# Nesquiko/Latticeum

Measured on AMD Instinct MI355X. Metric: fold-steps/sec (Ajtai commit+fold) at d=1024, higher is better.
Workload: dtype u64 (Goldilocks mod-p integer); 1 GPU; configs[2] at d=1024: commit+fold step, X^1024+1, W=16384, kappa=32, K=15; rho is an input; transcript, linearization, sumchecks, Mz outside the step; d=1024, W=16384, N=81920, kappa=32

## Files before the change

### latticeum_amd/csrc/ajtai_mfma.hip

```cpp
#include <cstdlib>
#include <cstring>

#include "frag.hpp"
#include "kernels.hpp"
#include "launch.hpp"

namespace lfk {

int mfma_dim(int d) { return d == 24 ? 40 : d; }

FragGeom frag_geom(size_t ncols, int Lp) {
  FragGeom g;
  g.Lp = Lp;
  g.Wp = ncols / Lp;
  const size_t nG = frag_groups(g.Wp);
  g.ptop = (int)frag_ptop(nG, Lp);
  g.nch = (int)(frag_npos(nG, Lp) / 2);
  return g;
}

template <bool VMAJOR, bool PHI72, bool ONEROW>
__global__ void __launch_bounds__(256) k_to_frag(VecPtrs rows, int rlo, int rhi, int d, int dv, int nch, int Lp,
                                                 size_t Wp, uint4 *frag, int qd) {
  __shared__ uint64_t tile[TF_R * TF_S * TF_J];
  const int sb = blockIdx.x, tid = threadIdx.x;
  const int c0 = ONEROW ? blockIdx.y * TF_R : blockIdx.y;
  const int r0 = ONEROW ? rlo : (rlo & ~(TF_R - 1)) + blockIdx.z * TF_R;
  if (PHI72) {
    const int r = tid >> 5, j = tid & 31;
    const int c = ONEROW ? c0 + r : c0, row = ONEROW ? r0 : r0 + r;
    bool ok;
    const size_t col = frag_column(c, j, Lp, Wp, ok);
    uint64_t ev[TF_S];
#pragma unroll
    for (int i = 0; i < TF_S; i++) ev[i] = 0;
    if (row >= rlo && row < rhi && c < nch && ok) {
      const uint64_t *e = rows.p[row] + col * d;
      if (sb == 0)
        phi72_evals<0>(e, ev);
      else if (sb == 1)
        phi72_evals<1>(e, ev);
      else
        phi72_evals<2>(e, ev);
    }
#pragma unroll
    for (int i = 0; i < TF_S; i++) tile[(r * TF_S + i) * TF_J + j] = VMAJOR ? fenc(ev[i]) : d8(ev[i]);
  } else {
#pragma unroll
    for (int it = 0; it < TF_R * 32 * 8 / 256; it++) {
      const int p = it * 256 + tid;
      const int r = p >> 8, j = (p >> 3) & 31, q = p & 7;
      const int c = ONEROW ? c0 + r : c0, row = ONEROW ? r0 : r0 + r;
      bool ok;
      const size_t col = frag_column(c, j, Lp, Wp, ok);
      ulonglong2 v = make_ulonglong2(0, 0);
      if (row >= rlo && row < rhi && c < nch && ok)
        v = *reinterpret_cast<const ulonglong2 *>(rows.p[row] + col * d + sb * TF_S + 2 * q);
      uint64_t *t = tile + (r * TF_S + 2 * q) * TF_J + j;
      t[0] = VMAJOR ? fenc(v.x) : d8(v.x);
      t[TF_J] = VMAJOR ? fenc(v.y) : d8(v.y);
    }
  }
  __syncthreads();
  const int r = tid & 7, h = (tid >> 3) & 1, sl = tid >> 4;
  const int c = ONEROW ? c0 + r : c0, row = ONEROW ? r0 : r0 + r;
  if (row < rlo || row >= rhi || c >= nch || sb * TF_S + sl >= dv) return;
  const ulonglong2 *src = reinterpret_cast<const ulonglong2 *>(tile + (r * TF_S + sl) * TF_J + 16 * h);
  uint64_t x[16];
#pragma unroll
  for (int q = 0; q < 8; q++) {
    const ulonglong2 t = src[q];
    x[2 * q] = t.x;
    x[2 * q + 1] = t.y;
  }
  uint4 u[8];
  d8_transpose16(x, u);
  const size_t s = op_slot((size_t)sb * TF_S + sl, qd);
  if (VMAJOR) {
    uint4 *out = frag + fv_index(s, nch, c, row, h);
#pragma unroll
    for (int b = 0; b < 8; b++) out[4 * b] = u[b];
  } else {
    uint4 *out = frag + ((s * nch + c) * 8) * 64 + row + 32 * h;
#pragma unroll
    for (int b = 0; b < 8; b++) out[b * 64] = u[b];
  }
}

constexpr int AJ_CPS = 320;
typedef __attribute__((address_space(3))) void lds_void;
__device__ __forceinline__ int fl_pi(int j, int i) { return i ^ (((j & 7) << 1) | ((i >> 5) & 1)); }

__device__ __forceinline__ void mfma_epilogue(const v16i *acc, int lane, int kt, int kappa, int nvec, int d, int so,
                                              int js, int direct, const OutPtrs &dst, uint64_t *partial,
                                              const uint64_t *kr) {
  const int v = lane & 31, h = lane >> 5;
  auto fe = [](int64_t x) { return x < 0 ? (uint64_t)x + gl::P : (uint64_t)x; };
#pragma unroll
  for (int i = 0; i < 16; i++) {
    int32_t x[15];
#pragma unroll
    for (int t = 0; t < 15; t++) x[t] = acc[t][i];
    asm volatile("" : "+v"(x[0]), "+v"(x[1]), "+v"(x[2]), "+v"(x[3]), "+v"(x[4]), "+v"(x[5]), "+v"(x[6]), "+v"(x[7]),
                 "+v"(x[8]), "+v"(x[9]), "+v"(x[10]), "+v"(x[11]), "+v"(x[12]), "+v"(x[13]), "+v"(x[14]));
    int64_t S[4] = {0, 0, 0, 0};
#pragma unroll
    for (int t = 0; t < 15; t++) S[t >> 2] += (int64_t)x[t] << (8 * (t & 3));
    uint64_t r = gl::add(fe(S[0] - S[2] - S[3]), gl::mul_pow2(fe(S[1] + S[2]), 32));
    const int row = 32 * kt + (i & 3) + 8 * (i >> 2) + 4 * h;
    if (v < nvec && row < kappa) {
      if (js == 0) r = gl::add(r, kr[(size_t)row * d + so]);
      if (direct)
        dst.p[v][(size_t)row * d + so] = r;
      else
        partial[(((size_t)js * nvec + v) * kappa + row) * d + so] = r;
    }
  }
}
__device__ __forceinline__ void mfma_epilogue_top(const v16i *acc, int lane, int kt, int kappa, int d, int so,
                                                  bool add_kr, uint64_t *out, const uint64_t *kr) {
  const int h = lane >> 5;
  auto fe = [](int64_t x) { return x < 0 ? (uint64_t)x + gl::P : (uint64_t)x; };
#pragma unroll
  for (int i = 0; i < 16; i++) {
    int32_t x[15];
#pragma unroll
    for (int t = 0; t < 15; t++) x[t] = acc[t][i];
    asm volatile("" : "+v"(x[0]), "+v"(x[1]), "+v"(x[2]), "+v"(x[3]), "+v"(x[4]), "+v"(x[5]), "+v"(x[6]), "+v"(x[7]),
                 "+v"(x[8]), "+v"(x[9]), "+v"(x[10]), "+v"(x[11]), "+v"(x[12]), "+v"(x[13]), "+v"(x[14]));
    int64_t S[4] = {0, 0, 0, 0};
#pragma unroll
    for (int t = 0; t < 15; t++) S[t >> 2] += (int64_t)x[t] << (8 * (t & 3));
    uint64_t r = gl::add(fe(S[0] - S[2] - S[3]), gl::mul_pow2(fe(S[1] + S[2]), 32));
    const int row = 32 * kt + (i & 3) + 8 * (i >> 2) + 4 * h;
    if (out && row < kappa) {
      if (add_kr) r = gl::add(r, kr[(size_t)row * d + so]);
      out[(size_t)row * d + so] = r;
    }
  }
}

template <int N>
__device__ __forceinline__ void vm_wait() {
  static_assert(N >= 0 && N < 64, "vmcnt is 6 bits");
  asm volatile("s_waitcnt vmcnt(%0)" ::"n"(N) : "memory");
}
template <int DP>
__device__ __forceinline__ void vm_wait_chunk(int nf) {
  switch (nf) {
    case 8: vm_wait<8 + (DP - 2) * 16>(); break;
    case 7: vm_wait<8 + (DP - 2) * 15>(); break;
    case 6: vm_wait<8 + (DP - 2) * 14>(); break;
    case 5: vm_wait<8 + (DP - 2) * 13>(); break;
    case 4: vm_wait<8 + (DP - 2) * 12>(); break;
    case 3: vm_wait<8 + (DP - 2) * 11>(); break;
    case 2: vm_wait<8 + (DP - 2) * 10>(); break;
    case 1: vm_wait<8 + (DP - 2) * 9>(); break;
    default: vm_wait<8 + (DP - 2) * 8>(); break;
  }
}
__device__ __forceinline__ void lgkm_wait_digit(int kb) {
  switch (kb) {
    case 0: asm volatile("s_waitcnt lgkmcnt(7)" ::: "memory"); break;
    case 1: asm volatile("s_waitcnt lgkmcnt(6)" ::: "memory"); break;
    case 2: asm volatile("s_waitcnt lgkmcnt(5)" ::: "memory"); break;
    case 3: asm volatile("s_waitcnt lgkmcnt(4)" ::: "memory"); break;
    case 4: asm volatile("s_waitcnt lgkmcnt(3)" ::: "memory"); break;
    case 5: asm volatile("s_waitcnt lgkmcnt(2)" ::: "memory"); break;
    case 6: asm volatile("s_waitcnt lgkmcnt(1)" ::: "memory"); break;
    default: asm volatile("s_waitcnt lgkmcnt(0)" ::: "memory"); break;
  }
}
template <int CPOL>
__device__ __forceinline__ v4i gload16(const v4i *p) {
  v4i r;
  if (CPOL == 2)
    asm volatile("global_load_dwordx4 %0, %1, off nt" : "=v"(r) : "v"(p) : "memory");
  else
    asm volatile("global_load_dwordx4 %0, %1, off" : "=v"(r) : "v"(p) : "memory");
  return r;
}
template <class T>
__device__ __forceinline__ T *uniform_ptr(T *p) {
  const uint64_t x = (uint64_t)(uintptr_t)p;
  const uint32_t lo = __builtin_amdgcn_readfirstlane((uint32_t)x), hi = __builtin_amdgcn_readfirstlane((uint32_t)(x >> 32));
  return reinterpret_cast<T *>((uintptr_t)(((uint64_t)hi << 32) | lo));
}
template <int CPA, int CPF, int DP, bool TOP>
__global__ void __launch_bounds__(256, 1) k_ajtai_mfma_ra(const uint4 *Af, const uint64_t *kr, StepOps so_, int nsteps,
                                                         int d, int nch,
                                                         int nvec, int kappa, int direct, int cps, int ktiles,
                                                         int nbase, size_t tile_u4, int qd, int clo, int chi, int pl0,
                                                         const uint32_t *tbl) {
  static_assert(DP >= 3 && DP <= 5, "F buffers: DP x 32 KiB of LDS");
  __shared__ uint4 Fl[DP][32 * 64];
  const int tid = threadIdx.x, lane = tid & 63, w = tid >> 6;
  const int per = 8 * ktiles * nsteps;
  const int grp = blockIdx.x / per, rem = blockIdx.x - grp * per;
  const int stp = rem / (8 * ktiles), rem2 = rem - stp * 8 * ktiles;
  const int kt = rem2 >> 3, bi = grp * 8 + (rem2 & 7);
  if (bi >= nbase) return;
  int nent = 0;
  if (TOP) {
    nent = top_tile_entries(tbl[0], stp, nsteps);
    if (nent == 0) return;
  }
  const uint4 *Ff = so_.Ff[TOP ? 0 : stp];
  uint64_t *partial = so_.partial[TOP ? 0 : stp];
  const OutPtrs &dst = so_.dst[TOP ? 0 : stp];
  const int gw = bi * 4 + w;
  const int s = gw % d, js = gw / d;
  if (js >= (chi - clo + cps - 1) / cps) return;
  const int c0 = clo + js * cps, c1 = min(chi, c0 + cps);
  v16i acc[15];
#pragma unroll
  for (int t = 0; t < 15; t++) acc[t] = (v16i){0};
  const v4i *pa = reinterpret_cast<const v4i *>(Af + kt * tile_u4 + ((size_t)s * nch * 8) * 64 + lane);
  const uint4 *ft = Ff + (size_t)(s >> 2) * nch * FV_CHUNK;
  v4i ra[DP][8];
  auto load_a = [&](int c, v4i *dstr) {
#pragma unroll
    for (int k = 0; k < 8; k++) {
      dstr[k] = gload16<CPA>(pa + ((size_t)c * 8 + k) * 64);
    }
  };
  const int nrow = TOP ? nent : nvec;
  const int nf = __builtin_amdgcn_readfirstlane((nrow - w + 3) >> 2 < 8 ? (nrow - w + 3) >> 2 : 8);
  const uint4 *ftq[8];
  const uint8_t *flq[8];
  if (TOP) {
    const int wu = __builtin_amdgcn_readfirstlane(w);
    const size_t quad = (size_t)__builtin_amdgcn_readfirstlane(s >> 2) * nch * FV_CHUNK;
#pragma unroll
    for (int q = 0; q < 8; q++) {
      const uint32_t e = __builtin_amdgcn_readfirstlane(tbl[1 + 32 * stp + 4 * q + wu]);
      const int est = top_step(e, nsteps), er = top_row(e);
      const uint4 *f = so_.Ff[0];
      DeadUnits du = so_.dead[0];
#pragma unroll
      for (int k = 1; k < LF_MAX_STEPS; k++) {
        f = est == k ? so_.Ff[k] : f;
        du.flags = est == k ? so_.dead[k].flags : du.flags;
        du.rows = est == k ? so_.dead[k].rows : du.rows;
      }
      ftq[q] = uniform_ptr(f + quad + (size_t)er * 64);
      flq[q] = uniform_ptr(du.flags && ((du.rows >> er) & 1u) ? du.flags + er : (const uint8_t *)nullptr);
    }
  }
  constexpr int NDM = (AJ_CPS + 63) / 64;
  const DeadUnits du = so_.dead[TOP ? 0 : stp];
  const bool has_dead = TOP || (du.flags != nullptr && du.rows != 0);
  uint32_t dm[NDM];
#pragma unroll
  for (int m = 0; m < NDM; m++) dm[m] = 0;
  if (TOP) {
#pragma unroll
    for (int m = 0; m < NDM; m++) {
      const int c = c0 + lane + 64 * m;
      if (c < c1) {
        uint32_t bits = 0;
#pragma unroll
        for (int q = 0; q < 8; q++)
          if (q < nf && flq[q])
            bits |= ((uint32_t)(flq[q][(size_t)c * 64] & 1u) << (2 * q)) |
                    ((uint32_t)(flq[q][(size_t)c * 64 + 32] & 1u) << (2 * q + 1));
        dm[m] = bits;
      }
    }
  } else if (has_dead) {
#pragma unroll
    for (int m = 0; m < NDM; m++) {
      const int c = c0 + lane + 64 * m;
      if (c < c1) {
        const uint4 *p = reinterpret_cast<const uint4 *>(du.flags + (size_t)c * 64);
        const uint4 a0 = p[0], a1 = p[1], b0 = p[2], b1 = p[3];
        const uint32_t ua[8] = {a0.x, a0.y, a0.z, a0.w, a1.x, a1.y, a1.z, a1.w};
        const uint32_t ub[8] = {b0.x, b0.y, b0.z, b0.w, b1.x, b1.y, b1.z, b1.w};
        uint32_t bits = 0;
#pragma unroll
        for (int q = 0; q < 8; q++)
          if ((du.rows >> (4 * q + w)) & 1)
            bits |= (((ua[q] >> (8 * w)) & 1u) << (2 * q)) | (((ub[q] >> (8 * w)) & 1u) << (2 * q + 1));
        dm[m] = bits;
      }
    }
  }
  auto dead_mask = [&](int c) -> uint32_t {
    if (!has_dead) return 0u;
    const int ci = c - c0, m = ci >> 6, l = ci & 63;
    uint32_t r = __builtin_amdgcn_readlane(dm[0], l);
#pragma unroll
    for (int k = 1; k < NDM; k++) {
      const uint32_t x = __builtin_amdgcn_readlane(dm[k], l);
      r = m == k ? x : r;
    }
    return r;
  };
  const int hl = lane >> 5;
  const uint4 *z80 = so_.zero80 + (lane & 31);
  auto stage_f = [&](int c, int buf) {
    const uint32_t dmask = dead_mask(c);
#pragma unroll
    for (int q = 0; q < 8; q++) {
      const int j = 4 * q + w;
      const uint4 *live = TOP ? ftq[q] + (size_t)c * FV_CHUNK + fl_pi(j, lane)
                              : ft + (size_t)c * FV_CHUNK + j * 64 + fl_pi(j, lane);
      const uint4 *src = ((dmask >> (2 * q + hl)) & 1u) ? z80 : live;
      if (q < nf) __builtin_amdgcn_global_load_lds((const void *)src, (lds_void *)&Fl[buf][j * 64], 16, 0, CPF);
    }
  };
  auto stage_f_piece = [&](int c, int buf, int q, uint32_t dmask) {
    const int j = 4 * q + w;
    const uint4 *live = TOP ? ftq[q] + (size_t)c * FV_CHUNK + fl_pi(j, lane)
                            : ft + (size_t)c * FV_CHUNK + j * 64 + fl_pi(j, lane);
    const uint4 *src = ((dmask >> (2 * q + hl)) & 1u) ? z80 : live;
    __builtin_amdgcn_global_load_lds((const void *)src, (lds_void *)&Fl[buf][j * 64], 16, 0, CPF);
  };
  const int rh = 2 * (lane & 31) + (lane >> 5), fj = rh >> 1;
  int fpos[8];
#pragma unroll
  for (int k = 0; k < 8; k++) fpos[k] = fj * 64 + fl_pi(fj, (rh & 1) * 32 + k * 4 + w);
#pragma unroll
  for (int j = 0; j < DP; j++) {
    if (c0 + j < c1) load_a(c0 + j, ra[j]);
    if (j < DP - 1 && c0 + j < c1) stage_f(c0 + j, j);
  }
  for (int cb = c0; cb < c1; cb += DP) {
#pragma unroll
    for (int j = 0; j < DP; j++) {
      const int c = cb + j;
      if (c >= c1) continue;
      if (c + DP - 1 < c1)
        vm_wait_chunk<DP>(nf);
      else
        vm_wait<0>();
      __builtin_amdgcn_s_barrier();
      v4i b[8];
      const uint32_t fbase = (uint32_t)(uintptr_t)&Fl[j][0];
#pragma unroll
      for (int k = 0; k < 8; k++) asm volatile("ds_read_b128 %0, %1" : "=v"(b[k]) : "v"(fbase + 16u * fpos[k]));
      const bool more_f = c + DP - 1 < c1, more_a = c + DP < c1;
      const int fb = (j + DP - 1) % DP;
      const uint32_t dmn = more_f ? dead_mask(c + DP - 1) : 0u;
#pragma unroll
      for (int kb = 0; kb < 8; kb++) {
        lgkm_wait_digit(kb);
        asm volatile("" : "+v"(b[kb]));
        if (kb == 0) {
#pragma unroll
          for (int k = 0; k < 8; k++) asm volatile("" : "+v"(ra[j][k]));
        }
        if (kb < 7) {
#pragma unroll
          for (int ka = 0; ka < 8; ka++)
            acc[ka + kb] = __builtin_amdgcn_mfma_i32_32x32x32_i8(ra[j][ka], b[kb], acc[ka + kb], 0, 0, 0);
          __builtin_amdgcn_sched_barrier(0);
          if (more_f && kb < nf) stage_f_piece(c + DP - 1, fb, kb, dmn);
          __builtin_amdgcn_sched_barrier(0);
        } else {
          if (more_f && nf == 8) stage_f_piece(c + DP - 1, fb, 7, dmn);
          __builtin_amdgcn_sched_barrier(0);
#pragma unroll
          for (int ka = 0; ka < 8; ka++) {
            acc[ka + 7] = __builtin_amdgcn_mfma_i32_32x32x32_i8(ra[j][ka], b[7], acc[ka + 7], 0, 0, 0);
            __builtin_amdgcn_sched_barrier(0);
            if (more_a) ra[j][ka] = gload16<CPA>(pa + ((size_t)(c + DP) * 8 + ka) * 64);
            __builtin_amdgcn_sched_barrier(0);
          }
        }
      }
    }
  }
  const int so = qd ? (s % qd) * 4 + s / qd : s;
  if (TOP) {
    const int v = lane & 31;
    const uint32_t e = tbl[1 + 32 * stp + v];
    const int est = top_step(e, nsteps), er = top_row(e);
    uint64_t *pp = so_.partial[0];
#pragma unroll
    for (int k = 1; k < LF_MAX_STEPS; k++) pp = est == k ? so_.partial[k] : pp;
    uint64_t *out = v < nent && er < nvec ? pp + ((size_t)(pl0 + js) * nvec + er) * kappa * d : nullptr;
    mfma_epilogue_top(acc, lane, kt, kappa, d, so, js == 0, out, kr);
  } else {
    mfma_epilogue(acc, lane, kt, kappa, nvec, d, so, js, direct, dst, partial, kr);
  }
}

__global__ void __launch_bounds__(512) k_fold_frag(const uint4 *frag, int nch, int Lp, size_t Wp, FoldRows fr,
                                                  const uint64_t *rho, int d, size_t N, uint64_t *out,
                                                  const int *run_if, int qd) {
  if (run_if && !*run_if) return;
  __shared__ uint64_t red[512 * 9];
  fold_frag_block<8>(blockIdx.x, frag, nch, Lp, Wp, fr, rho, d, N, out, red, qd);
}

hipError_t fold_frag(const uint4 *frag, const FragGeom &g, const FoldRows &fr, const uint64_t *rho, int d, size_t N,
                     uint64_t *out, hipStream_t st, const int *run_if) {
  if (d == 24 || d % 16 || fr.n < 1 || fr.n > LF_MAX_VECS) return hipErrorInvalidValue;
  if (!N) return hipSuccess;
  const size_t nb = (size_t)(d / 16) * g.nch;
  hipLaunchKernelGGL(k_fold_frag, dim3((unsigned)nb), dim3(512), 0, st, frag, g.nch, g.Lp, g.Wp, fr, rho, d, N, out,
                     run_if, g.qperm ? d / 4 : 0);
  return hipGetLastError();
}

__global__ void k_phi72_interp(const uint64_t *virt, int nvec, size_t kappa, OutPtrs out) {
  const size_t i = blockIdx.x * (size_t)blockDim.x + threadIdx.x;
  if (i >= (size_t)nvec * kappa * 8) return;
  const int slot = (int)(i & 7);
  const size_t vr = i >> 3, v = vr / kappa, row = vr - v * kappa;
  const uint64_t *P = virt + vr * 40 + 5 * slot;
  constexpr uint64_t INV2 = 0x7FFFFFFF80000001ull, INV3 = 0xAAAAAAAA00000001ull;
  const uint64_t d0 = P[0], d4 = P[4];
  const uint64_t d2 = gl::sub(gl::sub(gl::mul(gl::add(P[1], P[2]), INV2), d0), d4);
  const uint64_t s1 = gl::mul(gl::sub(P[1], P[2]), INV2);
  const uint64_t u =
      gl::mul(gl::sub(gl::sub(gl::sub(P[3], d0), gl::mul_pow2(d2, 2)), gl::mul_pow2(d4, 4)), INV2);
  const uint64_t d3 = gl::mul(gl::sub(u, s1), INV3), d1 = gl::sub(s1, d3);
  uint64_t *o = out.p[v] + row * 24 + 3 * slot;
  o[0] = gl::add(d0, gl::mul_pow2(d3, 40));
  o[1] = gl::add(d1, gl::mul_pow2(d4, 40));
  o[2] = d2;
}

__global__ void k_rowsum(const uint64_t *A, size_t kappa, size_t ncols, int d, uint64_t *tmp, size_t j0, size_t jstep) {
  const size_t t = blockIdx.x * (size_t)blockDim.x + threadIdx.x;
  if (t >= kappa * (size_t)d) return;
  const size_t i = t / d;
  const int w = (int)(t - i * d);
  const uint64_t *p = A + i * ncols * d + w;
  gl::Acc a;
  gl::acc_zero(a);
  for (size_t j = j0; j < ncols; j += jstep) gl::acc_add(a, p[j * d]);
  tmp[t] = gl::acc_reduce(a);
}
__global__ void k_kr_sub(const uint64_t *a, const uint64_t *b, size_t n, uint64_t *out) {
  const size_t t = blockIdx.x * (size_t)blockDim.x + threadIdx.x;
  if (t < n) out[t] = gl::sub(a[t], b[t]);
}
__global__ void k_rowsum_kr(const uint64_t *tmp, size_t kappa, int d, int dv, uint64_t *kr) {
  const size_t t = blockIdx.x * (size_t)blockDim.x + threadIdx.x;
  if (t >= kappa * (size_t)dv) return;
  const size_t i = t / dv;
  const int vs = (int)(t - i * dv);
  const uint64_t r = d == 24 ? ring::phi72_eval(tmp + i * 24, vs) : tmp[i * d + vs];
  kr[t] = gl::mul(FOFF, r);
}
size_t ajtai_rowsums_elems(size_t kappa, int d, int Lp) { return (Lp > 1 ? 3 : 1) * kappa * (size_t)mfma_dim(d); }
hipError_t ajtai_rowsums(const uint64_t *A, size_t kappa, size_t ncols, int d, uint64_t *kr, uint64_t *tmp,
                         hipStream_t st, int Lp) {
  const size_t n = kappa * (size_t)d, m = kappa * (size_t)mfma_dim(d);
  const dim3 gn(blocks(n, 256)), gm(blocks(m, 256));
  hipLaunchKernelGGL(k_rowsum, gn, dim3(256), 0, st, A, kappa, ncols, d, tmp, (size_t)0, (size_t)1);
  hipLaunchKernelGGL(k_rowsum_kr, gm, dim3(256), 0, st, tmp, kappa, d, mfma_dim(d), kr);
  if (Lp > 1) {
    hipLaunchKernelGGL(k_rowsum, gn, dim3(256), 0, st, A, kappa, ncols, d, tmp, (size_t)(Lp - 1), (size_t)Lp);
    hipLaunchKernelGGL(k_rowsum_kr, gm, dim3(256), 0, st, tmp, kappa, d, mfma_dim(d), kr + 2 * m);
    hipLaunchKernelGGL(k_kr_sub, gm, dim3(256), 0, st, kr, kr + 2 * m, m, kr + m);
  }
  return hipGetLastError();
}

struct StepDead {
  DeadUnits d[LF_MAX_STEPS];
};
__global__ void __launch_bounds__(1024) k_top_list(StepDead sd, int nsteps, int nvec, int ptop, int nG, uint32_t *tbl) {
  __shared__ uint32_t live[LF_MAX_STEPS];
  const int tid = threadIdx.x, q = tid & 7, gp = tid >> 3;
  if (tid < LF_MAX_STEPS) live[tid] = 0;
  __syncthreads();
#pragma unroll
  for (int s = 0; s < LF_MAX_STEPS; s++) {
    if (s >= nsteps) break;
    const DeadUnits du = sd.d[s];
    uint32_t lv = 0xFu << (4 * q);
    if (du.flags) {
      uint32_t a = 0x01010101u;
      for (int G = gp; G < nG; G += 128)
        a &= *reinterpret_cast<const uint32_t *>(du.flags + ((size_t)ptop + G) * 32 + 4 * q);
      uint32_t deadb = 0;
#pragma unroll
      for (int b = 0; b < 4; b++) deadb |= ((a >> (8 * b)) & 1u) << (4 * q + b);
      lv &= ~(deadb & du.rows);
    }
    if (lv) atomicOr(&live[s], lv);
  }
  __syncthreads();
  if (tid == 0) (void)top_compact(live, nsteps, nvec, tbl);
}

size_t frag_elems(const FragGeom &g, int d) { return (size_t)mfma_dim(d) * g.nch * 8 * 64; }
int mfma_ktiles(size_t kappa) { return (int)((kappa + 31) / 32); }
int mfma_cps(const FragGeom &g, int d) {
  const int dv = mfma_dim(d);
  if (dv >= 256) return AJ_CPS;
  const int want = 1024 / dv > 1 ? 1024 / dv : 1;
  const int cps = (g.nch + want - 1) / want;
  return cps < 1 ? 1 : (cps > AJ_CPS ? AJ_CPS : cps);
}
int mfma_nsplit(const FragGeom &g, int d) {
  const int cps = mfma_cps(g, d);
  return (g.nch + cps - 1) / cps;
}
struct ClassSplit {
  int cps, nsplit;
};
static ClassSplit class_split(int n, int cps_max) {
  const int ns = (n + cps_max - 1) / cps_max;
  return {ns ? (n + ns - 1) / ns : 1, ns};
}
static size_t mfma_planes(const FragGeom &g, int d) {
  const size_t nsplit = mfma_nsplit(g, d), whole = nsplit > 1 ? nsplit : 0;
  if (!g.ptop) return whole;
  const int cm = mfma_cps(g, d);
  const size_t cls = class_split(g.ptop / 2, cm).nsplit + class_split(g.nch - g.ptop / 2, cm).nsplit;
  return whole > cls ? whole : cls;
}
size_t mfma_scratch_elems(const FragGeom &g, int d, size_t kappa, int nvec) {
  const size_t dv = mfma_dim(d);
  return mfma_planes(g, d) * nvec * kappa * dv + (d == 24 ? (size_t)nvec * kappa * dv : 0);
}

hipError_t to_frag(const VecPtrs &rows, int nrows, int row0, const FragGeom &g, int d, bool vmajor, uint4 *frag,
                   hipStream_t st) {
  const int dv = mfma_dim(d);
  if (nrows < 1 || row0 < 0 || row0 + nrows > 32 || (d != 24 && d % TF_S)) return hipErrorInvalidValue;
  VecPtrs abs{};
  for (int i = 0; i < nrows; i++) abs.p[row0 + i] = rows.p[i];
  const int qd = g.qperm ? d / 4 : 0;
  const int rhi = row0 + nrows, ztiles = (rhi + TF_R - 1) / TF_R - row0 / TF_R;
  const dim3 grid((dv + TF_S - 1) / TF_S, g.nch, ztiles);
#define LF_TF(VM, PH) \
  hipLaunchKernelGGL((k_to_frag<VM, PH, false>), grid, dim3(256), 0, st, abs, row0, rhi, d, dv, g.nch, g.Lp, g.Wp, frag, \
                     qd)
  if (nrows == 1 && vmajor) {
    const dim3 grid1((dv + TF_S - 1) / TF_S, (g.nch + TF_R - 1) / TF_R, 1);
    if (d == 24)
      hipLaunchKernelGGL((k_to_frag<true, true, true>), grid1, dim3(256), 0, st, abs, row0, rhi, d, dv, g.nch, g.Lp,
                         g.Wp, frag, qd);
    else
      hipLaunchKernelGGL((k_to_frag<true, false, true>), grid1, dim3(256), 0, st, abs, row0, rhi, d, dv, g.nch, g.Lp,
                         g.Wp, frag, qd);
    return hipGetLastError();
  }
  if (d == 24) {
    if (vmajor)
      LF_TF(true, true);
    else
      LF_TF(false, true);
  } else if (vmajor) {
    LF_TF(true, false);
  } else {
    LF_TF(false, false);
  }
#undef LF_TF
  return hipGetLastError();
}

hipError_t ajtai_mfma_steps(const uint4 *Af, const uint64_t *kr, size_t kappa, const FragGeom &g, int d, int nvec,
                            int nsteps,
                            const uint4 *const *Ff, uint64_t *const *partial, const OutPtrs *dst, hipStream_t st,
                            hipEvent_t ev0, hipEvent_t ev1, const DeadUnits *dead, const uint4 *zero80,
                            uint32_t *toptbl) {
  const int dv = mfma_dim(d);
  const int ktiles = mfma_ktiles(kappa);
  const char *tc = getenv("LATTICEUM_AMD_TOPCLASS");
  const size_t top_work = (size_t)(g.nch - g.ptop / 2) * dv * ktiles * (nsteps - 1);
  const bool topc = g.ptop > 0 && nsteps >= 2 && toptbl && zero80 && !(tc && tc[0] == '0') &&
                    ((tc && tc[0] == '1') || (nsteps >= 4 && top_work >= ((size_t)1 << 17)));
  bool any_dead = false;
  for (int s = 0; dead && s < nsteps && s < LF_MAX_STEPS; s++) any_dead |= dead[s].flags != nullptr;
  if (!kr || (any_dead && !zero80) || kappa < 1 || ktiles > LF_MAX_KTILES || nvec < 1 || nvec > 32 || dv % 4 || nsteps < 1 ||
      nsteps > LF_MAX_STEPS)
    return hipErrorInvalidValue;
  const int nsplit = mfma_nsplit(g, d), cps = mfma_cps(g, d);
  const size_t plane = (size_t)nvec * kappa * dv;
  StepOps so{};
  so.zero80 = zero80;
  for (int s = 0; s < nsteps; s++) {
    so.Ff[s] = Ff[s];
    so.partial[s] = partial[s];
    so.dst[s] = dst[s];
    if (dead && zero80) so.dead[s] = dead[s];
    if (d == 24) {
      uint64_t *virt = partial[s] + mfma_planes(g, d) * plane;
      for (int v = 0; v < nvec; v++) so.dst[s].p[v] = virt + (size_t)v * kappa * dv;
    }
  }
  if (ev0) (void)hipEventRecord(ev0, st);
  const size_t tile_u4 = frag_elems(g, d);
  const bool big = (size_t)dv * g.nch * 8192 > STREAM_OUT_BYTES;
  const int qd = g.qperm ? d / 4 : 0;
#define LF_AJ(CA, CF, TOPC, KR, SLOTS, DIRECT, CPS, NS, CLO, CHI, PL0)                                              \
  do {                                                                                                              \
    const int nbase_ = (int)(((size_t)dv * (NS) + 3) / 4);                                                          \
    const dim3 grid_((unsigned)((nbase_ + 7) / 8 * 8 * ktiles * (SLOTS)));                                          \
    hipLaunchKernelGGL((k_ajtai_mfma_ra<CA, CF, 4, TOPC>), grid_, dim3(256), 0, st, Af, KR, so, SLOTS, dv, g.nch,  \
                       nvec, (int)kappa, DIRECT, CPS, ktiles, nbase_, tile_u4, qd, CLO, CHI, PL0,                  \
                       (const uint32_t *)toptbl);                                                                   \
  } while (0)
  int nplanes = nsplit > 1 ? nsplit : 0;
  if (topc) {
    const int ctop = g.ptop / 2;
    const ClassSplit cf = class_split(ctop, cps), ct = class_split(g.nch - ctop, cps);
    const size_t m = (size_t)kappa * dv;
    StepDead sdd{};
    for (int s = 0; s < nsteps; s++) sdd.d[s] = so.dead[s];
    hipLaunchKernelGGL(k_top_list, dim3(1), dim3(1024), 0, st, sdd, nsteps, nvec, g.ptop, (int)frag_groups(g.Wp),
                       toptbl);
    for (int s = 0; s < nsteps; s++) {
      const hipError_t em = hipMemsetAsync(partial[s] + cf.nsplit * plane, 0, ct.nsplit * plane * sizeof(uint64_t), st);
      if (em != hipSuccess) return em;
    }
    if (big) {
      LF_AJ(0, 2, false, kr + m, nsteps, 0, cf.cps, cf.nsplit, 0, ctop, 0);
      LF_AJ(0, 2, true, kr + 2 * m, nsteps, 0, ct.cps, ct.nsplit, ctop, g.nch, cf.nsplit);
    } else {
      LF_AJ(0, 0, false, kr + m, nsteps, 0, cf.cps, cf.nsplit, 0, ctop, 0);
      LF_AJ(0, 0, true, kr + 2 * m, nsteps, 0, ct.cps, ct.nsplit, ctop, g.nch, cf.nsplit);
    }
    nplanes = cf.nsplit + ct.nsplit;
  } else {
    const int direct = nsplit == 1 ? 1 : 0;
    if (big && nsteps == 1)
      LF_AJ(2, 2, false, kr, nsteps, direct, cps, nsplit, 0, g.nch, 0);
    else if (big)
      LF_AJ(0, 2, false, kr, nsteps, direct, cps, nsplit, 0, g.nch, 0);
    else
      LF_AJ(0, 0, false, kr, nsteps, direct, cps, nsplit, 0, g.nch, 0);
  }
#undef LF_AJ
  hipError_t e = hipGetLastError();
  if (e != hipSuccess) return e;
  if (ev1) (void)hipEventRecord(ev1, st);
  for (int s = 0; s < nsteps; s++) {
    if (nplanes) {
      e = sum_planes_to(partial[s], nplanes, kappa * (size_t)dv, nvec, so.dst[s], st);
      if (e != hipSuccess) return e;
    }
    if (d == 24) {
      const size_t n = (size_t)nvec * kappa * 8;
      hipLaunchKernelGGL(k_phi72_interp, dim3(blocks(n, 256)), dim3(256), 0, st, so.dst[s].p[0], nvec,
                         kappa, dst[s]);
      e = hipGetLastError();
      if (e != hipSuccess) return e;
    }
  }
  return hipSuccess;
}

hipError_t ajtai_mfma(const uint4 *Af, const uint64_t *kr, size_t kappa, const FragGeom &g, int d, const VecPtrs &fv,
                      int nvec,
                      bool f_ready, uint4 *Ff, uint64_t *partial, uint64_t *cm, hipStream_t st, hipEvent_t ev0,
                      hipEvent_t ev1, const OutPtrs *dst, const DeadUnits *dead, const uint4 *zero80) {
  if (nvec < 1 || nvec > 32 || (!cm && !dst)) return hipErrorInvalidValue;
  OutPtrs out{};
  for (int v = 0; v < nvec; v++) out.p[v] = cm ? cm + (size_t)v * kappa * d : dst->p[v];
  if (!f_ready) {
    hipError_t e = to_frag(fv, nvec, 0, g, d, true, Ff, st);
    if (e != hipSuccess) return e;
  }
  const uint4 *ff[1] = {Ff};
  uint64_t *pp[1] = {partial};
  return ajtai_mfma_steps(Af, kr, kappa, g, d, nvec, 1, ff, pp, &out, st, ev0, ev1, f_ready ? dead : nullptr, zero80);
}

}
```

Measured before the change: 60.36 fold-steps/s.

## Specialize steady-state MFMA loop and cut address arithmetic in Ajtai kernel

Rewrites the inner loop of the MFMA Ajtai commit kernel to lower per-instruction scalar and vector overhead. A-tile loads now use an SGPR base plus immediate offsets. F staging writes m0 directly through inline asm with precomputed permutation offsets. The main loop is split into steady-state rounds, compile-time specialized for nf=8 and nf=7 with bounds checks removed, followed by a generic tail. It also merges the TOP dead-flag gathering into the pointer setup loop and adds an explicit waitcnt. These changes risk register pressure and correctness issues from hand-written m0 and LDS offset assumptions.

```diff
diff --git a/latticeum_amd/csrc/ajtai_mfma.hip b/latticeum_amd/csrc/ajtai_mfma.hip
--- a/latticeum_amd/csrc/ajtai_mfma.hip
+++ b/latticeum_amd/csrc/ajtai_mfma.hip
@@ -1,5 +1,7 @@
 #include <cstdlib>
 #include <cstring>
+#include <type_traits>
+#include <utility>
 
 #include "frag.hpp"
 #include "kernels.hpp"
@@ -171,14 +173,23 @@
     default: asm volatile("s_waitcnt lgkmcnt(0)" ::: "memory"); break;
   }
 }
-template <int CPOL>
-__device__ __forceinline__ v4i gload16(const v4i *p) {
+template <int CPOL, int OFF>
+__device__ __forceinline__ v4i gload16(const void *base, uint32_t voff) {
+  static_assert(OFF >= 0 && OFF < 4096, "immediate offset");
   v4i r;
   if (CPOL == 2)
-    asm volatile("global_load_dwordx4 %0, %1, off nt" : "=v"(r) : "v"(p) : "memory");
+    asm volatile("global_load_dwordx4 %0, %1, %2 offset:%3 nt" : "=v"(r) : "v"(voff), "s"(base), "n"(OFF) : "memory");
   else
-    asm volatile("global_load_dwordx4 %0, %1, off" : "=v"(r) : "v"(p) : "memory");
+    asm volatile("global_load_dwordx4 %0, %1, %2 offset:%3" : "=v"(r) : "v"(voff), "s"(base), "n"(OFF) : "memory");
   return r;
+}
+template <class F, int... I>
+__device__ __forceinline__ void static_for_seq(F &&f, std::integer_sequence<int, I...>) {
+  (f(std::integral_constant<int, I>{}), ...);
+}
+template <int N, class F>
+__device__ __forceinline__ void static_for(F &&f) {
+  static_for_seq(f, std::make_integer_sequence<int, N>{});
 }
 template <class T>
 __device__ __forceinline__ T *uniform_ptr(T *p) {
@@ -194,7 +205,8 @@
                                                          const uint32_t *tbl) {
   static_assert(DP >= 3 && DP <= 5, "F buffers: DP x 32 KiB of LDS");
   __shared__ uint4 Fl[DP][32 * 64];
-  const int tid = threadIdx.x, lane = tid & 63, w = tid >> 6;
+  const int tid = threadIdx.x, lane = tid & 63;
+  const int w = __builtin_amdgcn_readfirstlane(tid >> 6);
   const int per = 8 * ktiles * nsteps;
   const int grp = blockIdx.x / per, rem = blockIdx.x - grp * per;
   const int stp = rem / (8 * ktiles), rem2 = rem - stp * 8 * ktiles;
@@ -215,25 +227,30 @@
   v16i acc[15];
 #pragma unroll
   for (int t = 0; t < 15; t++) acc[t] = (v16i){0};
-  const v4i *pa = reinterpret_cast<const v4i *>(Af + kt * tile_u4 + ((size_t)s * nch * 8) * 64 + lane);
+  const uint4 *pa = Af + kt * tile_u4 + ((size_t)s * nch * 8) * 64;
+  const uint32_t va0 = 16u * lane, va1 = va0 + 4096u;
   const uint4 *ft = Ff + (size_t)(s >> 2) * nch * FV_CHUNK;
   v4i ra[DP][8];
-  auto load_a = [&](int c, v4i *dstr) {
-#pragma unroll
-    for (int k = 0; k < 8; k++) {
-      dstr[k] = gload16<CPA>(pa + ((size_t)c * 8 + k) * 64);
-    }
+  auto load_a_k = [&](int c, auto k_) __attribute__((always_inline)) -> v4i {
+    constexpr int k = decltype(k_)::value;
+    const uint4 *cb = pa + (size_t)c * 8 * 64;
+    return gload16<CPA, (k & 3) * 1024>(cb, k < 4 ? va0 : va1);
+  };
+  auto load_a = [&](int c, v4i *dstr) __attribute__((always_inline)) {
+    static_for<8>([&](auto k_) __attribute__((always_inline)) { dstr[decltype(k_)::value] = load_a_k(c, k_); });
   };
   const int nrow = TOP ? nent : nvec;
   const int nf = __builtin_amdgcn_readfirstlane((nrow - w + 3) >> 2 < 8 ? (nrow - w + 3) >> 2 : 8);
+  constexpr int NDM = (AJ_CPS + 63) / 64;
+  uint32_t dm[NDM];
+#pragma unroll
+  for (int m = 0; m < NDM; m++) dm[m] = 0;
   const uint4 *ftq[8];
-  const uint8_t *flq[8];
   if (TOP) {
-    const int wu = __builtin_amdgcn_readfirstlane(w);
-    const size_t quad = (size_t)__builtin_amdgcn_readfirstlane(s >> 2) * nch * FV_CHUNK;
+    const size_t quad = (size_t)(s >> 2) * nch * FV_CHUNK;
 #pragma unroll
     for (int q = 0; q < 8; q++) {
-      const uint32_t e = __builtin_amdgcn_readfirstlane(tbl[1 + 32 * stp + 4 * q + wu]);
+      const uint32_t e = __builtin_amdgcn_readfirstlane(tbl[1 + 32 * stp + 4 * q + w]);
       const int est = top_step(e, nsteps), er = top_row(e);
       const uint4 *f = so_.Ff[0];
       DeadUnits du = so_.dead[0];
@@ -244,30 +261,20 @@
         du.rows = est == k ? so_.dead[k].rows : du.rows;
       }
       ftq[q] = uniform_ptr(f + quad + (size_t)er * 64);
-      flq[q] = uniform_ptr(du.flags && ((du.rows >> er) & 1u) ? du.flags + er : (const uint8_t *)nullptr);
-    }
-  }
-  constexpr int NDM = (AJ_CPS + 63) / 64;
+      const uint8_t *fl = uniform_ptr(du.flags && ((du.rows >> er) & 1u) ? du.flags + er : (const uint8_t *)nullptr);
+      if (q < nf && fl) {
+#pragma unroll
+        for (int m = 0; m < NDM; m++) {
+          const int c = c0 + lane + 64 * m;
+          if (c < c1)
+            dm[m] |= ((uint32_t)(fl[(size_t)c * 64] & 1u) << (2 * q)) | ((uint32_t)(fl[(size_t)c * 64 + 32] & 1u) << (2 * q + 1));
+        }
+      }
+    }
+  }
   const DeadUnits du = so_.dead[TOP ? 0 : stp];
   const bool has_dead = TOP || (du.flags != nullptr && du.rows != 0);
-  uint32_t dm[NDM];
-#pragma unroll
-  for (int m = 0; m < NDM; m++) dm[m] = 0;
-  if (TOP) {
-#pragma unroll
-    for (int m = 0; m < NDM; m++) {
-      const int c = c0 + lane + 64 * m;
-      if (c < c1) {
-        uint32_t bits = 0;
-#pragma unroll
-        for (int q = 0; q < 8; q++)
-          if (q < nf && flq[q])
-            bits |= ((uint32_t)(flq[q][(size_t)c * 64] & 1u) << (2 * q)) |
-                    ((uint32_t)(flq[q][(size_t)c * 64 + 32] & 1u) << (2 * q + 1));
-        dm[m] = bits;
-      }
-    }
-  } else if (has_dead) {
+  if (!TOP && has_dead) {
 #pragma unroll
     for (int m = 0; m < NDM; m++) {
       const int c = c0 + lane + 64 * m;
@@ -285,8 +292,8 @@
       }
     }
   }
+  __builtin_amdgcn_s_waitcnt(0x0F70);
   auto dead_mask = [&](int c) -> uint32_t {
-    if (!has_dead) return 0u;
     const int ci = c - c0, m = ci >> 6, l = ci & 63;
     uint32_t r = __builtin_amdgcn_readlane(dm[0], l);
 #pragma unroll
@@ -298,23 +305,30 @@
   };
   const int hl = lane >> 5;
   const uint4 *z80 = so_.zero80 + (lane & 31);
-  auto stage_f = [&](int c, int buf) {
-    const uint32_t dmask = dead_mask(c);
-#pragma unroll
-    for (int q = 0; q < 8; q++) {
-      const int j = 4 * q + w;
-      const uint4 *live = TOP ? ftq[q] + (size_t)c * FV_CHUNK + fl_pi(j, lane)
-                              : ft + (size_t)c * FV_CHUNK + j * 64 + fl_pi(j, lane);
-      const uint4 *src = ((dmask >> (2 * q + hl)) & 1u) ? z80 : live;
-      if (q < nf) __builtin_amdgcn_global_load_lds((const void *)src, (lds_void *)&Fl[buf][j * 64], 16, 0, CPF);
-    }
+  const uint32_t pi0 = 16u * fl_pi(w, lane), pi1 = 16u * fl_pi(4 + w, lane);
+  const uint32_t lw0 = (uint32_t)(uintptr_t)&Fl[0][0] + 1024u * w;
+  auto stage_f_piece = [&](int c, int buf, int q, uint32_t dmv) __attribute__((always_inline)) {
+    const int j = 4 * q + w;
+    const uint4 *row = TOP ? ftq[q] + (size_t)c * FV_CHUNK : ft + (size_t)c * FV_CHUNK + j * 64;
+    const uint4 *live = reinterpret_cast<const uint4 *>(reinterpret_cast<const char *>(row) + ((q & 1) ? pi1 : pi0));
+    const uint4 *src = (dmv & (1u << (2 * q))) ? z80 : live;
+    if (CPF == 2)
+      asm volatile("s_add_i32 m0, %1, %2\n\ts_nop 0\n\tglobal_load_lds_dwordx4 %0, off nt"
+                   :: "v"(src), "s"(lw0), "i"((buf * 32 + 4 * q) * 1024) : "memory", "scc");
+    else
+      asm volatile("s_add_i32 m0, %1, %2\n\ts_nop 0\n\tglobal_load_lds_dwordx4 %0, off"
+                   :: "v"(src), "s"(lw0), "i"((buf * 32 + 4 * q) * 1024) : "memory", "scc");
   };
-  auto stage_f_piece = [&](int c, int buf, int q, uint32_t dmask) {
-    const int j = 4 * q + w;
-    const uint4 *live = TOP ? ftq[q] + (size_t)c * FV_CHUNK + fl_pi(j, lane)
-                            : ft + (size_t)c * FV_CHUNK + j * 64 + fl_pi(j, lane);
-    const uint4 *src = ((dmask >> (2 * q + hl)) & 1u) ? z80 : live;
-    __builtin_amdgcn_global_load_lds((const void *)src, (lds_void *)&Fl[buf][j * 64], 16, 0, CPF);
+  auto lane_mask = [&](uint32_t dmask) -> uint32_t {
+    uint32_t v = dmask >> hl;
+    asm volatile("" : "+v"(v));
+    return v;
+  };
+  auto stage_f = [&](int c, int buf) __attribute__((always_inline)) {
+    const uint32_t dmv = lane_mask(dead_mask(c));
+#pragma unroll
+    for (int q = 0; q < 8; q++)
+      if (q < nf) stage_f_piece(c, buf, q, dmv);
   };
   const int rh = 2 * (lane & 31) + (lane >> 5), fj = rh >> 1;
   int fpos[8];
@@ -325,23 +339,32 @@
     if (c0 + j < c1) load_a(c0 + j, ra[j]);
     if (j < DP - 1 && c0 + j < c1) stage_f(c0 + j, j);
   }
-  for (int cb = c0; cb < c1; cb += DP) {
+  auto round = [&](auto steady_, auto nfc_, int cb) __attribute__((always_inline)) {
+    constexpr bool STEADY = decltype(steady_)::value;
+    constexpr int NFC = decltype(nfc_)::value;
+    const int nfr = NFC >= 0 ? NFC : nf;
 #pragma unroll
     for (int j = 0; j < DP; j++) {
       const int c = cb + j;
-      if (c >= c1) continue;
-      if (c + DP - 1 < c1)
-        vm_wait_chunk<DP>(nf);
+      if (!STEADY && c >= c1) continue;
+      if (STEADY || c + DP - 1 < c1)
+        vm_wait_chunk<DP>(nfr);
       else
         vm_wait<0>();
       __builtin_amdgcn_s_barrier();
       v4i b[8];
-      const uint32_t fbase = (uint32_t)(uintptr_t)&Fl[j][0];
-#pragma unroll
-      for (int k = 0; k < 8; k++) asm volatile("ds_read_b128 %0, %1" : "=v"(b[k]) : "v"(fbase + 16u * fpos[k]));
-      const bool more_f = c + DP - 1 < c1, more_a = c + DP < c1;
+      const uint32_t fbase = (uint32_t)(uintptr_t)&Fl[j & ~1][0];
+#pragma unroll
+      for (int k = 0; k < 8; k++) {
+        if (j & 1)
+          asm volatile("ds_read_b128 %0, %1 offset:32768" : "=v"(b[k]) : "v"(fbase + 16u * fpos[k]));
+        else
+          asm volatile("ds_read_b128 %0, %1" : "=v"(b[k]) : "v"(fbase + 16u * fpos[k]));
+      }
+      const bool more_f = STEADY || c + DP - 1 < c1, more_a = STEADY || c + DP < c1;
       const int fb = (j + DP - 1) % DP;
-      const uint32_t dmn = more_f ? dead_mask(c + DP - 1) : 0u;
+      const uint32_t dmn = more_f ? lane_mask(dead_mask(c + DP - 1)) : 0u;
+      const int ncopy = more_f ? nfr : 0;
 #pragma unroll
       for (int kb = 0; kb < 8; kb++) {
         lgkm_wait_digit(kb);
@@ -355,22 +378,31 @@
           for (int ka = 0; ka < 8; ka++)
             acc[ka + kb] = __builtin_amdgcn_mfma_i32_32x32x32_i8(ra[j][ka], b[kb], acc[ka + kb], 0, 0, 0);
           __builtin_amdgcn_sched_barrier(0);
-          if (more_f && kb < nf) stage_f_piece(c + DP - 1, fb, kb, dmn);
+          if (kb < ncopy) stage_f_piece(c + DP - 1, fb, kb, dmn);
           __builtin_amdgcn_sched_barrier(0);
         } else {
-          if (more_f && nf == 8) stage_f_piece(c + DP - 1, fb, 7, dmn);
+          if (ncopy == 8) stage_f_piece(c + DP - 1, fb, 7, dmn);
           __builtin_amdgcn_sched_barrier(0);
-#pragma unroll
-          for (int ka = 0; ka < 8; ka++) {
+          static_for<8>([&](auto ka_) __attribute__((always_inline)) {
+            constexpr int ka = decltype(ka_)::value;
             acc[ka + 7] = __builtin_amdgcn_mfma_i32_32x32x32_i8(ra[j][ka], b[7], acc[ka + 7], 0, 0, 0);
             __builtin_amdgcn_sched_barrier(0);
-            if (more_a) ra[j][ka] = gload16<CPA>(pa + ((size_t)(c + DP) * 8 + ka) * 64);
+            if (more_a) ra[j][ka] = load_a_k(c + DP, ka_);
             __builtin_amdgcn_sched_barrier(0);
-          }
+          });
         }
       }
     }
-  }
+  };
+  using steady_t = std::integral_constant<bool, true>;
+  using tail_t = std::integral_constant<bool, false>;
+  int cb = c0;
+  int is8 = nf == 8, is7 = nf == 7;
+  asm volatile("" : "+v"(is8), "+v"(is7));
+  is8 = __builtin_amdgcn_readfirstlane(is8), is7 = __builtin_amdgcn_readfirstlane(is7);
+  for (; is8 && cb + 2 * DP - 1 < c1; cb += DP) round(steady_t{}, std::integral_constant<int, 8>{}, cb);
+  for (; is7 && cb + 2 * DP - 1 < c1; cb += DP) round(steady_t{}, std::integral_constant<int, 7>{}, cb);
+  for (; cb < c1; cb += DP) round(tail_t{}, std::integral_constant<int, -1>{}, cb);
   const int so = qd ? (s % qd) * 4 + s / qd : s;
   if (TOP) {
     const int v = lane & 31;
```

Result: faster. 62.57 fold-steps/s, median of 6 (+3.7%).
